# elador/FeatureDetection

Hardware: AMD Instinct MI355X
Metric: Mpatches/s (extract+WVM+SVM) per GPU, 640x480 pyramid (higher is better)
Workload: dtype u8/i32/f32/f64; 1 GPU; config 1/metric config: ffpDetectApp FaceFrontal.cfg five-stage cascade on 640x480 BGR frames: 13-layer pyramid, 20x20 windows step 1 (16185 windows/frame), HistEq64 -> WVM 280 filters -> OE -> RBF-SVM 1024 SV -> NMS; fd_pyramid_update_frames + fd_detect_five_stage_frames (the frames of a call share one pyramid aren...; frames_per_call=64, calls_in_flight=11, parallelism=image-shard dp1

## Files before the change

### featuredetection_amd/capi.py

```python
import ctypes as C
import os
import numpy as np

_HERE = os.path.dirname(os.path.abspath(__file__))
LIB_PATH = os.environ.get("FD_HIP_LIB", os.path.join(_HERE, "libfd_hip.so"))

FD_OK, FD_ERR_INVALID_ARGUMENT, FD_ERR_RUNTIME, FD_ERR_LOGIC, FD_ERR_HIP, FD_ERR_CAPACITY, FD_ERR_DEVICE_CAPACITY = range(7)
FD_LAYER_NONE, FD_LAYER_GRADBIN, FD_LAYER_LBP = 0, 1, 2
IMAGE_GRAY, IMAGE_GREYWORLD_GRAY = 0, 1
FD_KERNEL_LINEAR, FD_KERNEL_POLY, FD_KERNEL_RBF, FD_KERNEL_HIK = 0, 1, 2, 3
FD_DTYPE_U8, FD_DTYPE_F32 = 0, 1


class FdError(RuntimeError):
    def __init__(self, code, msg):
        super().__init__("fd_hip error %d: %s" % (code, msg))
        self.code = code


class fd_wvm_model(C.Structure):
    _fields_ = [("filter_w", C.c_int32), ("filter_h", C.c_int32), ("num_filters", C.c_int32), ("num_used", C.c_int32),
                ("num_per_level", C.c_int32), ("basis_param", C.c_float), ("bias", C.c_float),
                ("thresholds", C.POINTER(C.c_float)), ("hk_weights", C.POINTER(C.c_float)), ("pp", C.POINTER(C.c_double)),
                ("val_off", C.POINTER(C.c_int32)), ("val", C.POINTER(C.c_double)), ("rec_off", C.POINTER(C.c_int32)),
# ... 310 lines not shown
    "fd_integral_update": (C.c_int, [C.c_void_p, C.c_void_p, C.c_int, C.c_int, C.c_int, C.c_int]),
    "fd_integral_set_image": (C.c_int, [C.c_void_p, C.c_void_p, C.c_int, C.c_int]),
    "fd_integral_size": (C.c_int, [C.c_void_p, C.POINTER(C.c_int), C.POINTER(C.c_int)]),
    "fd_integral_download": (C.c_int, [C.c_void_p, C.c_void_p]),
    "fd_integral_image": (C.c_int, [C.c_void_p, C.c_void_p, C.c_int, C.c_int, C.c_void_p]),
    "fd_haar_grid": (C.c_int, [C.c_int, C.c_void_p]),
    "fd_haar_feature_count": (C.c_int, [C.POINTER(fd_haar_params)]),
    "fd_haar_features": (C.c_int, [C.POINTER(fd_haar_params), C.c_void_p, C.c_int, C.POINTER(C.c_int)]),
    "fd_integral_extract_haar": (C.c_int, [C.c_void_p, C.c_void_p, C.POINTER(fd_haar_params), C.c_int, C.c_void_p, C.c_void_p, C.c_void_p]),
    "fd_integral_gradient_patches": (C.c_int, [C.c_void_p, C.c_void_p, C.c_int, C.c_int, C.c_int, C.c_void_p, C.c_void_p, C.c_void_p]),
    "fd_gradient_sum_batch": (C.c_int, [C.c_void_p, C.c_void_p, C.c_int64, C.c_int, C.c_int, C.c_int, C.c_int, C.c_void_p]),
    "fd_integral_extract_surf": (C.c_int, [C.c_void_p, C.c_void_p, C.c_int, C.c_int, C.c_int, C.c_void_p, C.c_void_p, C.c_void_p]),
    "fd_integral_svm_evaluate_samples": (C.c_int, [C.c_void_p, C.c_void_p, C.c_int, C.c_void_p, C.c_void_p, C.c_int, C.c_void_p, C.c_void_p,
                                                   C.c_void_p]),
    "fd_integral_image_length": (C.c_int, [C.c_int, C.c_int]),
    "fd_integral_gradient_length": (C.c_int, [C.c_int, C.c_int]),
    "fd_gradient_sum_length": (C.c_int, [C.c_int, C.c_int, C.c_int, C.c_int]),
    "fd_surf_feature_length": (C.c_int, [C.c_int, C.c_int]),
}

_BENCH_SIGS = {
    "fd_debug_svm_u8_both": (C.c_int, [C.c_void_p, C.c_void_p, C.c_void_p, C.c_int64, C.c_void_p, C.c_void_p]),
    "fd_ctx_set_kernel_timing": (C.c_int, [C.c_void_p, C.c_int]),
    "fd_last_kernel_ms": (C.c_int, [C.c_void_p, C.POINTER(C.c_char_p), C.POINTER(C.c_float)]),
    "fd_last_group_prefilter_ms": (C.c_int, [C.c_void_p, C.POINTER(C.c_float), C.POINTER(C.c_int)]),
    "fd_debug_wvb_rect_sums": (C.c_int64, [C.POINTER(fd_wvm_model), C.c_void_p, C.c_int64, C.c_void_p, C.c_void_p]),
    "fd_wvm_last_queue_length": (C.c_int64, [C.c_void_p]),
    "fd_wvm_last_tail_state": (C.c_int, [C.c_void_p]),
    "fd_wvm_last_spec_state": (C.c_int, [C.c_void_p]),
    "fd_wvm_last_stage_b_plan": (C.c_int, [C.c_void_p, C.c_void_p]),
    "fd_debug_wvd_plan": (C.c_int, [C.c_void_p, C.c_void_p, C.c_int, C.c_int, C.c_int, C.c_int, C.c_int, C.c_void_p]),
    "fd_debug_wvd_packed_plan": (C.c_int, [C.c_void_p, C.c_void_p, C.c_int, C.c_int, C.c_int, C.c_int, C.c_int, C.c_void_p, C.c_void_p, C.c_void_p,
                                           C.c_int64, C.c_void_p]),
}


def lib():
    global _lib
    if _lib is None:
        if not os.path.exists(LIB_PATH):
            raise ImportError("%s not built: run `python -c 'import __graft_entry__ as g; g.build()'` "
                              "(hipcc --offload-arch=gfx950); there is no CPU fallback" % LIB_PATH)
        l = C.CDLL(LIB_PATH)
        for name, (res, args) in list(_SIGS.items()) + list(_BENCH_SIGS.items()):
            f = getattr(l, name)
            f.restype = res
            f.argtypes = args
        _lib = l
    return _lib


def _ptr(a):
    return a.ctypes.data_as(C.c_void_p) if a is not None else None


def _c(arr, dtype):
    return np.ascontiguousarray(arr, dtype=dtype)


class Context:
    def __init__(self, device=0, stream=None):
        self.h = C.c_void_p()
        rc = lib().fd_ctx_create(device, C.c_void_p(stream) if stream else None, C.byref(self.h))
        if rc != FD_OK:
            raise FdError(rc, "fd_ctx_create failed (no usable gfx950 device?)")

# ... 265 lines not shown
    dist.ctx.check(lib().fd_dist_gather_records(dist.h, _ptr(local), len(local), cap, None, 0, C.byref(n), C.byref(tr)))
    return int(n.value)


def svm_u8_both(ctx, svm, feats):
    feats = _c(feats, np.uint8).reshape(-1, svm.dim)
    o8, o16 = np.empty(len(feats), np.float64), np.empty(len(feats), np.float64)
    ctx.check(lib().fd_debug_svm_u8_both(ctx.h, svm.h, _ptr(feats), len(feats), _ptr(o8), _ptr(o16)))
    return o8, o16


def wvd_plan(nx, ny, frames, sy, ph, slots):
    nx, ny = _c(nx, np.int32), _c(ny, np.int32)
    first = np.zeros(len(nx) + 1, np.int32)
    k = lib().fd_debug_wvd_plan(_ptr(nx), _ptr(ny), len(nx), frames, sy, ph, slots, _ptr(first))
    if k < 1:
        raise FdError(k, "fd_debug_wvd_plan")
    return k, first


def wvd_packed_plan(nx, ny, frames, sy, ph, slots, tasks=None):
    nx, ny = _c(nx, np.int32), _c(ny, np.int32)
    tiles, ntask = C.c_int32(), C.c_int32()
    k = lib().fd_debug_wvd_packed_plan(_ptr(nx), _ptr(ny), len(nx), frames, sy, ph, slots, C.byref(tiles), C.byref(ntask), None, 0, None)
    if k < 1:
        raise FdError(k, "fd_debug_wvd_packed_plan")
    tasks = np.arange(ntask.value, dtype=np.int32) if tasks is None else _c(tasks, np.int32)
    dec = np.zeros((len(tasks), 4), np.int32)
    if len(tasks):
        k = lib().fd_debug_wvd_packed_plan(_ptr(nx), _ptr(ny), len(nx), frames, sy, ph, slots, None, None, _ptr(tasks), len(tasks), _ptr(dec))
        if k < 1:
            raise FdError(k, "fd_debug_wvd_packed_plan")
    return k, tiles.value, ntask.value, dec


def wvb_rect_sums(model, patches_eq):
    s, keep = _wvm_struct(model, fd_wvm_model)
    patches_eq = _c(patches_eq, np.uint8)
    n = patches_eq.shape[0]
    gen = np.zeros(5, np.int32)
    ncols = lib().fd_debug_wvb_rect_sums(C.byref(s), None, 0, None, _ptr(gen))
    if ncols < 0:
        return None
    out = np.empty((n, ncols), np.int32)
    lib().fd_debug_wvb_rect_sums(C.byref(s), _ptr(patches_eq), n, _ptr(out), None)
    return out, [int(g) for g in gen if g >= 0]


def wvm_eval(ctx, wvm, patches_eq):
    patches_eq = _c(patches_eq, np.uint8)
    n = patches_eq.shape[0]
    lv = np.empty(n, np.int32)
    sc = np.empty(n, np.float32)
    ctx.check(lib().fd_wvm_eval_batch(ctx.h, wvm.h, _ptr(patches_eq), n, _ptr(lv), _ptr(sc)))
    return lv, sc


class Svm:
    def __init__(self, ctx, model):
        self.ctx = ctx
        self.model = model
        dtype = np.uint8 if model["dtype"] == FD_DTYPE_U8 else np.float32
        sv = _c(model["sv"], dtype)
        coeff = _c(model["coeff"], np.float32)
        s = fd_svm_model()
        s.kernel = int(model["kernel"])
# ... 1193 lines not shown
```

### featuredetection_amd/csrc/pyramid.hip

```cpp
#include "fd_internal.hpp"
#include "fd_device.hpp"
#include <algorithm>
#include <cstring>

namespace {

constexpr int MAXJ = 16;

struct ResizeJob {
    int dw, dh;
    uint32_t dst_off;
    double scale_x, scale_y;
};
struct ResizeJobs {
    int n;
    ResizeJob j[MAXJ];
};
struct DownJob {
    int sw, sh;
    uint32_t src_off, dst_off;
};
struct FusedJob {
    int dw0, dh0, dw1, dh1;
    uint32_t dst0_off;
    uint32_t dst1_off;
    uint32_t xtab;
    double scale_y;
};
struct FusedJobs {
    int n;
    FusedJob j[MAXJ];
};
struct DownJobs {
    int n;
    int tile0[MAXJ + 1];
    DownJob j[MAXJ];
};
struct FilterJob {
    int w, h;
    uint32_t src_off, dst_off;
};
struct FilterJobs {
    int n;
    FilterJob j[MAXJ];
};

__device__ __forceinline__ int reflect101(int p, int len) {
    if (len == 1) return 0;
    while (p < 0 || p >= len) {
        if (p < 0) p = -p;
        else p = 2 * len - 2 - p;
    }
    return p;
}
__device__ __forceinline__ int reflect1(int p, int len) {
    if (len < 3) return reflect101(p, len);
    const int q = p < 0 ? -p : (p >= len ? 2 * len - 2 - p : p);
    return min(max(q, 0), len - 1);
}

struct FramePtrs {
    const uint8_t* p[FD_MAX_FRAMES];
};
__device__ __forceinline__ unsigned int mul24(unsigned int a, unsigned int b) {
    unsigned int r;
    asm("v_mul_u32_u24 %0, %1, %2" : "=v"(r) : "v"(a), "v"(b));
    return r;
}
__device__ __forceinline__ unsigned int mul24_s(unsigned int a_uniform, unsigned int b) {
    unsigned int r;
// ... 42 lines not shown
            uint32_t w[GQ][3];
#pragma unroll
            for (int i = 0; i < GQ; ++i) load3(min(q + i * stride, nq - 1), w[i]);
#pragma unroll
            for (int i = 0; i < GQ; ++i)
                if (q + i * stride < nq) reinterpret_cast<uint32_t*>(gray)[q + i * stride] = gray4(w[i]);
        } else {
            uint32_t w[GQ];
#pragma unroll
            for (int i = 0; i < GQ; ++i) w[i] = ld_u32_unaligned(src + 4 * (size_t)min(q + i * stride, nq - 1));
#pragma unroll
            for (int i = 0; i < GQ; ++i)
                if (q + i * stride < nq) reinterpret_cast<uint32_t*>(gray)[q + i * stride] = w[i];
        }
    }
    if (blockIdx.x == 0 && (int)threadIdx.x < (n & 3)) {
        const int i = (nq << 2) + threadIdx.x;
        gray[i] = ch == 3 ? (uint8_t)gray_of(src[3 * (size_t)i], src[3 * (size_t)i + 1], src[3 * (size_t)i + 2]) : src[i];
    }
}

__global__ void k_bgr2gray(const uint8_t* __restrict__ bgr, uint8_t* __restrict__ gray, int n) {
    int i = blockIdx.x * blockDim.x + threadIdx.x;
    int stride = gridDim.x * blockDim.x;
    for (; i < n; i += stride) {
        int b = bgr[3 * (size_t)i], g = bgr[3 * (size_t)i + 1], r = bgr[3 * (size_t)i + 2];
        gray[i] = (uint8_t)((b * 1868 + g * 9617 + r * 4899 + 8192) >> 14);
    }
}

constexpr int TL_W = 64, TL_H = 32, TL_PITCH = 136;
constexpr int PD_TH = 16;
constexpr int TL_ROWS = 72;

__global__ __launch_bounds__(256) void k_resize_tiled(const uint8_t* __restrict__ arena, uint8_t* __restrict__ out, uint32_t src_off, int sw,
                                                      int sh, ResizeJobs jobs, size_t imageStride) {
    __shared__ __attribute__((aligned(16))) uint8_t tile[TL_ROWS * TL_PITCH];
    __shared__ int4 rowTab[TL_H];
    const ResizeJob jb = jobs.j[blockIdx.y];
    const uint8_t* src = arena + (size_t)blockIdx.z * imageStride + src_off;
    uint8_t* dst = out + (size_t)blockIdx.z * imageStride + jb.dst_off;
    const int tilesX = (jb.dw + TL_W - 1) / TL_W, tilesY = (jb.dh + TL_H - 1) / TL_H;
    auto srcX = [&](int dx, float& fx) {
        fx = (float)((dx + 0.5) * jb.scale_x - 0.5);
        int sx = (int)floorf(fx);
        fx -= sx;
        if (sx < 0) { fx = 0; sx = 0; }
        if (sx >= sw - 1) { fx = 0; sx = sw - 1; }
        return sx;
    };
    auto srcY = [&](int dy, float& fy) {
        fy = (float)((dy + 0.5) * jb.scale_y - 0.5);
        const int sy = (int)floorf(fy);
        fy -= sy;
        return sy;
    };
    auto clampY = [&](int y) { return y < 0 ? 0 : (y >= sh ? sh - 1 : y); };
    const int c = threadIdx.x & 63, rq = __builtin_amdgcn_readfirstlane(threadIdx.x >> 6);
    for (int t = blockIdx.x; t < tilesX * tilesY; t += gridDim.x) {
        const int ty = t / tilesX, tx = t - ty * tilesX;
        const int dx0 = tx * TL_W, dy0 = ty * TL_H;
        const int X0 = max(0, (int)((float)dx0 * (float)jb.scale_x) - 1), Y0 = max(0, (int)((float)dy0 * (float)jb.scale_y) - 1);
        {
            const int x = X0 + 4 * c;
            const bool colok = c < TL_PITCH / 4;
            uint32_t v[TL_ROWS / 4];
// ... 130 lines not shown
        if (itemN < items)
            fused_issue(f, arena0 + (size_t)frame_of(itemN) * imageStride + src_off, sw, sh, tabs, jobs.j[dN.w], dN);
        PYR_T(p3);
        {
            const int c = threadIdx.x & 127, half = __builtin_amdgcn_readfirstlane(threadIdx.x >> 7);
            if (c < G0_W) {
                const int rBase = half * (G0_H - 18);
                const int lx = min(max(ex.x - X0, 0), FS_PITCH - 1) + 2 * rBase * FS_PITCH;
                int lx1 = lx + 1;
                asm("" : "+v"(lx1));
                const uint8_t *sp = stage + lx, *sp1 = stage + lx1;
                const uint2* tp = taps + rBase;
                const u16x2 aw = __builtin_bit_cast(u16x2, ex.y);
                uint8_t* gp = g0 + rBase * G0_PITCH + c;
#pragma unroll
                for (int i = 0; i < 18; ++i) {
                    const uint8_t *s = sp + 2 * i * FS_PITCH, *s1 = sp1 + 2 * i * FS_PITCH;
                    const u16x2 p0 = {s[0], s1[0]}, p1 = {s[FS_PITCH], s1[FS_PITCH]};
                    const uint2 t = tp[i];
                    const unsigned int h0 = __builtin_amdgcn_udot2(p0, aw, 0u, false) & ~15u;
                    const unsigned int h1 = __builtin_amdgcn_udot2(p1, aw, 0u, false) & ~15u;
                    gp[i * G0_PITCH] = (uint8_t)((mulhi24(t.x, h0) + mulhi24(t.y, h1) + 2) >> 2);
                }
            }
        }
        PYR_T(p4);
        __syncthreads();
        PYR_T(p5);
        {
            const int c1 = lane;
            const int x = x1 + c1;
            if (c1 < FT_W1 && x < jb.dw1) {
                constexpr int PR = FT_H1 / 4;
                const uint8_t* T = g0 + (2 * wave * PR) * G0_PITCH + 2 * c1;
                int h[2 * PR + 3];
#pragma unroll
                for (int r = 0; r < 2 * PR + 3; ++r) {
                    const uint8_t* S = T + r * G0_PITCH;
                    const uint32_t p01 = *reinterpret_cast<const uint16_t*>(S), p23 = *reinterpret_cast<const uint16_t*>(S + 2);
                    h[r] = (int)__builtin_amdgcn_udot4(p01 | (p23 << 16), 0x04060401u, (uint32_t)S[4], false);
                }
                uint8_t* dp = arena + jb.dst1_off + (uint32_t)((y1 + wave * PR) * jb.dw1) + x;
#pragma unroll
                for (int j = 0; j < PR; ++j, dp += jb.dw1) {
                    if (y1 + wave * PR + j < jb.dh1) {
                        const int v = h[2 * j + 2] * 6 + (h[2 * j + 1] + h[2 * j + 3]) * 4 + h[2 * j] + h[2 * j + 4];
                        *dp = (uint8_t)((v + 128) >> 8);
                    }
                }
            }
        }
        if (jb.dst0_off != 0xffffffffu) {
            uint8_t* d0 = arena + jb.dst0_off;
            for (int i = threadIdx.x; i < 32 * 128; i += 256) {
                const int r = 2 + (i >> 7), c = 2 + (i & 127);
                const int gx = gx0 + c, gy = gy0 + r;
                if (c < 2 + 2 * FT_W1 && gx < jb.dw0 && gy < jb.dh0) d0[(uint32_t)(gy * jb.dw0) + gx] = g0[r * G0_PITCH + c];
            }
        }
#ifdef FD_PYR_PROF
        {
            const unsigned long long p6 = __builtin_amdgcn_s_memtime();
            pacc[0] += p1 - p0; pacc[1] += p2 - p1; pacc[2] += p3 - p2; pacc[3] += p4 - p3; pacc[4] += p5 - p4; pacc[5] += p6 - p5; ++ptiles;
        }
#endif
    }
#ifdef FD_PYR_PROF
    if (threadIdx.x == 0 && blockIdx.x < (unsigned int)PYR_PROF_WGS) {
        for (int i = 0; i < 6; ++i) fd_pyr_prof[blockIdx.x * 8 + i] = pacc[i];
        fd_pyr_prof[blockIdx.x * 8 + 6] = ptiles;
    }
#endif
}

__device__ __forceinline__ int reflect_cf(int p, int len) {
    int q = p < 0 ? -p : p;
    q = q >= len ? 2 * len - 2 - q : q;
    return min(max(q, 0), len - 1);
}
constexpr int PD_W = 62;
__global__ __launch_bounds__(256) void k_pyrdown_tiled(uint8_t* __restrict__ arena0, DownJobs jobs, size_t imageStride, int xcdFrames) {
    __shared__ __attribute__((aligned(16))) uint8_t tile[TL_ROWS * TL_PITCH];
    const int c = threadIdx.x & 63, rq = __builtin_amdgcn_readfirstlane(threadIdx.x >> 6);
    constexpr int NROWS = 2 * PD_TH + 3, PD_LD = (NROWS + 7) / 8;
    static_assert(2 * (3 + 4 * (PD_LD - 1)) + 1 < TL_ROWS && 128 <= TL_PITCH && 2 * PD_W + 3 <= 128, "pyrDown stage");
    const bool byXcd = xcdFrames > 0;
    const int ntile = jobs.tile0[jobs.n];
    const int first = byXcd ? (int)(blockIdx.x >> 3) : (int)blockIdx.x, stride = byXcd ? (int)(gridDim.x >> 3) : (int)gridDim.x;
    const int items = byXcd ? (xcdFrames >> 3) * ntile : ntile;
    for (int item = first; item < items; item += stride) {
        const int fi = byXcd ? item / ntile : 0;
        const int g = item - fi * ntile;
        uint8_t* __restrict__ arena = arena0 + (size_t)(byXcd ? (int)(blockIdx.x & 7u) + 8 * fi : (int)blockIdx.z) * imageStride;
        int ji = 0;
        while (ji + 1 < jobs.n && g >= jobs.tile0[ji + 1]) ++ji;
        const DownJob jb = jobs.j[ji];
        const int t = g - jobs.tile0[ji];
        const int sw = jb.sw, sh = jb.sh;
        const int dw = (sw + 1) / 2, dh = (sh + 1) / 2;
        const uint8_t* src = arena + jb.src_off;
        uint8_t* dst = arena + jb.dst_off;
        const int tilesX = (dw + PD_W - 1) / PD_W;
        const int ty = t / tilesX, tx = t - ty * tilesX;
        const int dx0 = tx * PD_W, dy0 = ty * PD_TH;
        const int X0 = 2 * dx0 - 2, Y0 = 2 * dy0 - 2;
        {
            const int j4 = 4 * (c & 31), half = c >> 5;
            const int xs = X0 + j4;
            const int xc = min(max(xs, 0), max(sw - 4, 0));
            const uint32_t lastDw = (uint32_t)max(sw * sh - 4, 0);
            uint32_t v[PD_LD];
#pragma unroll
            for (int k = 0; k < PD_LD; ++k) {
                const int r = 2 * (rq + 4 * k) + half;
                v[k] = ld_u32_unaligned(src + min((uint32_t)(reflect_cf(Y0 + r, sh) * sw + xc), lastDw));
            }
            if (X0 < 0 || X0 + 128 > sw) {
                if (!(xs >= 0 && xs + 3 < sw)) {
#pragma unroll
                    for (int k = 0; k < PD_LD; ++k) {
                        const int r = 2 * (rq + 4 * k) + half;
                        const uint8_t* row = src + (uint32_t)(reflect_cf(Y0 + r, sh) * sw);
                        uint32_t w = 0;
#pragma unroll
                        for (int b = 0; b < 4; ++b) w |= (uint32_t)row[reflect_cf(xs + b, sw)] << (8 * b);
                        v[k] = w;
                    }
                }
            }
#pragma unroll
            for (int k = 0; k < PD_LD; ++k) *reinterpret_cast<uint32_t*>(&tile[(2 * (rq + 4 * k) + half) * TL_PITCH + j4]) = v[k];
        }
        __syncthreads();
        const int x = dx0 + c;
        if (c < PD_W && x < dw) {
            constexpr int PR = PD_TH / 4;
            const uint8_t* T = tile + (2 * rq * PR) * TL_PITCH + 2 * c;
            int h[2 * PR + 3];
#pragma unroll
            for (int r = 0; r < 2 * PR + 3; ++r) {
                const uint8_t* S = T + r * TL_PITCH;
                const uint32_t p01 = *reinterpret_cast<const uint16_t*>(S), p23 = *reinterpret_cast<const uint16_t*>(S + 2);
                h[r] = (int)__builtin_amdgcn_udot4(p01 | (p23 << 16), 0x04060401u, (uint32_t)S[4], false);
            }
            uint8_t* dp = dst + (uint32_t)((dy0 + rq * PR) * dw) + x;
#pragma unroll
            for (int j = 0; j < PR; ++j, dp += dw) {
                if (dy0 + rq * PR + j < dh) {
                    const int v = h[2 * j + 2] * 6 + (h[2 * j + 1] + h[2 * j + 3]) * 4 + h[2 * j] + h[2 * j + 4];
                    *dp = (uint8_t)((v + 128) >> 8);
                }
            }
        }
        __syncthreads();
    }
}

__device__ __forceinline__ float grad_pair(const uint8_t* __restrict__ src, int w, int h, int x, int y, int ksize, int& gx, int& gy) {
    if (ksize == 1 || ksize == 3) {
        const int xm = reflect101(x - 1, w), xp = reflect101(x + 1, w);
        const int ym = reflect101(y - 1, h), yp = reflect101(y + 1, h);
        const uint8_t *S0 = src + (size_t)ym * w, *S1 = src + (size_t)y * w, *S2 = src + (size_t)yp * w;
        if (ksize == 1) {
            gx = S1[xp] - S1[xm];
            gy = S2[x] - S0[x];
            return 0.5f;
        }
        gx = (S0[xp] - S0[xm]) + 2 * (S1[xp] - S1[xm]) + (S2[xp] - S2[xm]);
        gy = (S2[xm] - S0[xm]) + 2 * (S2[x] - S0[x]) + (S2[xp] - S0[xp]);
        return 0.125f;
    }
    int a, d1, d2, d3, s0, s1, s2, s3;
    float scale;
    if (ksize == 5) { a = 2; d1 = 2; d2 = 1; d3 = 0; s0 = 6; s1 = 4; s2 = 1; s3 = 0; scale = 1.f / 128.f; }
    else if (ksize == 7) { a = 3; d1 = 5; d2 = 4; d3 = 1; s0 = 20; s1 = 15; s2 = 6; s3 = 1; scale = 1.f / 2048.f; }
    else { a = 1; d1 = 1; d2 = 0; d3 = 0; s0 = 10; s1 = 3; s2 = 0; s3 = 0; scale = 1.f / 32.f; }
    const int dk[4] = {0, d1, d2, d3}, sk[4] = {s0, s1, s2, s3};
    int cx[7], cy[7];
    for (int t = -a; t <= a; ++t) { cx[t + a] = reflect101(x + t, w); cy[t + a] = reflect101(y + t, h); }
    gx = 0;
    gy = 0;
    for (int j = -a; j <= a; ++j) {
        const uint8_t* S = src + (size_t)cy[j + a] * w;
        int rd = 0, rs = 0;
        for (int i = 1; i <= a; ++i) {
            const int hi = S[cx[a + i]], lo = S[cx[a - i]];
            rd += dk[i] * (hi - lo);
// ... 292 lines not shown
                if (direction < 0) direction += PI;
                bin = direction * bins / PI;
            }
            auto sat = [](double v) { int r = fd_cvRound(v); return (uint8_t)(r < 0 ? 0 : (r > 255 ? 255 : r)); };
            size_t index = (size_t)x | ((size_t)y << 8);
            if (!interpolate) {
                lut[2 * index] = (uint8_t)((uint8_t)std::round(bin) % (unsigned)bins);
                lut[2 * index + 1] = sat(255 * magnitude);
            } else {
                uint8_t w1 = sat(255 * magnitude * (bin - std::floor(bin)));
                lut[4 * index] = (uint8_t)((uint8_t)std::floor(bin) % (unsigned)bins);
                lut[4 * index + 1] = sat(255 * magnitude - w1);
                lut[4 * index + 2] = (uint8_t)((uint8_t)std::ceil(bin) % (unsigned)bins);
                lut[4 * index + 3] = w1;
            }
        }
    }
}

int grid_for(int npix) { return std::max(1, std::min(1024, (npix + 255) / 256)); }
int tile_grid_for(int ntiles) { return std::max(1, std::min(1024, ntiles)); }

struct ResizeLaunch {
    ResizeJobs jobs;
    int grid;
};
struct FusedLaunch {
    FusedJobs jobs;
    uint32_t tileTab;
    int tilesPerFrame;
    int grid;
};
struct DownLaunch {
    DownJobs jobs;
};
struct FilterLaunch {
    FilterJobs jobs, blur;
    int grid;
};

}

struct fd_pyramid::Plan {
    std::vector<ResizeLaunch> resize;
    std::vector<FusedLaunch> fused;
    std::vector<DownLaunch> down;
    std::vector<FilterLaunch> filter;
};
fd_pyramid::~fd_pyramid() { if (ready) (void)hipEventDestroy(ready); }

namespace {

template <class Launch>
auto& next_job(std::vector<Launch>& launches, size_t first = 0) {
    if (launches.size() == first || launches.back().jobs.n == MAXJ) launches.emplace_back();
    auto& jobs = launches.back().jobs;
    return jobs.j[jobs.n++];
}

void build_plan(fd_pyramid* p, int W, int H) {
    p->plan.reset(new fd_pyramid::Plan());
    fd_pyramid::Plan& plan = *p->plan;
    const std::vector<HostLayer>& all = p->all;
    const int NI = p->nimg;
    static const int mode = [] { const char* e = getenv("FD_PYR_FUSED"); return e ? atoi(e) : 1; }();
    std::vector<char> fused(all.size(), 0);
    std::vector<int2> tab;
    std::vector<std::vector<int4>> tiles;
    for (size_t k = 0; k < all.size(); ++k) {
        const HostLayer& L = all[k];
        if (L.depth != 0) continue;
        if (L.w == W && L.h == H && L.gray_off == p->gray_full_off) continue;
        const double scale_x = 1. / ((double)L.w / W), scale_y = 1. / ((double)L.h / H);
        if (!(scale_x >= 1.0 && scale_x <= 2.05 && scale_y >= 1.0 && scale_y <= 2.05))
            FD_THROW(FD_ERR_RUNTIME, "ImagePyramid: first-octave layer %d x %d of a %d x %d image is outside the resize kernel's range", L.w, L.h, W, H);
        const bool chain = k + 1 < all.size() && all[k + 1].depth == 1 && all[k + 1].chain == L.chain;
        if (chain && mode != 0 && (!L.kept || mode == 2) && L.w >= 3 && L.h >= 3 && W <= 65535 && H <= 65535) {
            const HostLayer& D = all[k + 1];
            std::vector<int2> xt((size_t)L.w);
            for (int dx = 0; dx < L.w; ++dx) {
                float fx = (float)((dx + 0.5) * scale_x - 0.5);
                int sx = (int)floorf(fx);
                fx -= sx;
                if (sx < 0) { fx = 0; sx = 0; }
                if (sx >= W - 1) { fx = 0; sx = W - 1; }
                const int a0 = (int)nearbyintf((1.f - fx) * 2048), a1 = (int)nearbyintf(fx * 2048);
                xt[(size_t)dx] = make_int2(sx, a0 | (a1 << 16));
            }
// ... 11 lines not shown
                j.scale_y = scale_y;
                tab.insert(tab.end(), xt.begin(), xt.end());
                tiles.resize(plan.fused.size());
                for (int ty = 0; ty * FT_H1 < D.h; ++ty)
                    for (int tx = 0; tx * FT_W1 < D.w; ++tx) {
                        const int gx0 = 2 * tx * FT_W1 - 2;
                        const int cLo = std::max(0, gx0), cHi = std::min(L.w - 1, gx0 + G0_W - 1);
                        const int X0 = xt[(size_t)cLo].x, ncol = std::min(W - 1, xt[(size_t)cHi].x + 1) - X0 + 1;
                        tiles.back().push_back(make_int4(X0, ncol, (int)((uint32_t)tx | (uint32_t)ty << 16), plan.fused.back().jobs.n - 1));
                    }
                fused[k] = 1;
                continue;
            }
        }
        ResizeJob& j = next_job(plan.resize);
        j.dw = L.w; j.dh = L.h; j.dst_off = L.gray_off;
        j.scale_x = scale_x;
        j.scale_y = scale_y;
        ResizeLaunch& R = plan.resize.back();
        R.grid = std::max(R.grid, tile_grid_for(((L.w + TL_W - 1) / TL_W) * ((L.h + TL_H - 1) / TL_H)));
    }
    if (!plan.fused.empty()) {
        int perCu = 0;
        if (hipOccupancyMaxActiveBlocksPerMultiprocessor(&perCu, k_resize_down, 256, 0) != hipSuccess || perCu < 1) perCu = 4;
        for (size_t g = 0; g < plan.fused.size(); ++g) {
            FusedLaunch& F = plan.fused[g];
            if (tab.size() & 1) tab.push_back(make_int2(0, 0));
            F.tileTab = (uint32_t)tab.size();
            F.tilesPerFrame = (int)tiles[g].size();
            for (const int4& t : tiles[g]) { tab.push_back(make_int2(t.x, t.y)); tab.push_back(make_int2(t.z, t.w)); }
            F.grid = (int)std::min<int64_t>((int64_t)F.tilesPerFrame * NI, (int64_t)p->ctx->num_cus * perCu);
            if (NI >= 8 && F.grid >= 64) F.grid &= ~7;
        }
        p->rtab.reserve(sizeof(int2) * tab.size());
        HIP_CHECK(hipMemcpy(p->rtab.p, tab.data(), sizeof(int2) * tab.size(), hipMemcpyHostToDevice));
    }
    int maxDepth = 0;
    for (const HostLayer& L : all) maxDepth = std::max(maxDepth, L.depth);
    for (int d = 1; d <= maxDepth; ++d) {
        const size_t first = plan.down.size();
        for (size_t k = 1; k < all.size(); ++k) {
            const HostLayer& L = all[k];
            if (L.depth != d || fused[k - 1]) continue;
            const HostLayer& S = all[k - 1];
            DownJob& j = next_job(plan.down, first);
            j.sw = S.w; j.sh = S.h; j.src_off = S.gray_off; j.dst_off = L.gray_off;
            DownJobs& jobs = plan.down.back().jobs;
            jobs.tile0[jobs.n] = jobs.tile0[jobs.n - 1] + ((L.w + PD_W - 1) / PD_W) * ((L.h + PD_TH - 1) / PD_TH);
        }
    }
    if (p->filter_kind != FD_LAYER_NONE) {
        const bool blur = p->filter_kind == FD_LAYER_GRADBIN && p->grad_blur > 0;
        for (int k : p->kept) {
            const HostLayer& L = all[k];
            FilterJob& j = next_job(plan.filter);
            j.w = L.w; j.h = L.h; j.src_off = blur ? L.blur_off : L.gray_off; j.dst_off = L.filt_off;
            FilterLaunch& F = plan.filter.back();
            if (blur) {
                FilterJob& b = F.blur.j[F.blur.n++];
                b.w = L.w; b.h = L.h; b.src_off = L.gray_off; b.dst_off = L.blur_off;
            }
            F.grid = std::max(F.grid, grid_for(L.w * L.h));
        }
    }
}

void invalidate_layout(fd_pyramid* p) {
    p->all.clear();
    p->img_w = p->img_h = 0;
}

void build_layout(fd_pyramid* p, int W, int H) {
    invalidate_layout(p);
    p->kept.clear();
    size_t off = 0;
    p->gray_full_off = 0;
    off = align256((size_t)W * H);
    const int fch = p->filter_kind == FD_LAYER_GRADBIN ? (p->interpolate ? 4 : 2) : 1;
    for (size_t i = 0; i < p->octl; ++i) {
        double scaleFactor = std::pow(p->inc, (double)i);
        int w = fd_cvRound(W * scaleFactor), h = fd_cvRound(H * scaleFactor);
        if (w < 1 || h < 1) FD_THROW(FD_ERR_INVALID_ARGUMENT, "ImagePyramid: layer %zu would be empty", i);
// ... 65 lines not shown
    const size_t IS = p->image_stride;
    FramePtrs fp{};
    if (!is_device) p->input.reserve(bytes * NI);
    for (int f = 0; f < NI; ++f) {
        fp.p[f] = frames ? frames[f] : image;
        if (!is_device) {
            uint8_t* staged = p->input.as<uint8_t>() + (size_t)f * bytes;
            HIP_CHECK(hipMemcpyAsync(staged, fp.p[f], bytes, hipMemcpyHostToDevice, st));
            fp.p[f] = staged;
        }
    }
    if (greyworld) {
        GwStats* stats = p->gw_stats.as<GwStats>();
        HIP_CHECK(hipMemsetAsync(stats, 0, sizeof(GwStats) * (size_t)NI, st));
        const int cus = std::max(1, p->ctx->num_cus);
        const int perFrame = std::max(1, std::min(cus, 4 * cus / NI));
        const int gx = std::max(1, std::min((int)((npix / 4 + 1023) / 1024), perFrame));
        hipLaunchKernelGGL(k_gw_stats, dim3(gx, NI), dim3(256), 0, st, fp, stats, (int)npix);
        hipLaunchKernelGGL(k_gw_gray, dim3(gx, NI), dim3(256), 0, st, fp, stats, gray, IS, (int)npix);
    } else if (frames) {
        hipLaunchKernelGGL(k_frames_to_gray, dim3(grid_for((int)(npix / 16 + 1)), NI), dim3(256), 0, st, fp, gray, IS, (int)npix, ch);
    } else if (ch == 3) {
        hipLaunchKernelGGL(k_bgr2gray, dim3(grid_for((int)npix)), dim3(256), 0, st, fp.p[0], gray, (int)npix);
    } else {
        HIP_CHECK(hipMemcpyAsync(gray, fp.p[0], npix, hipMemcpyDeviceToDevice, st));
    }
    const fd_pyramid::Plan& plan = *p->plan;
    for (const ResizeLaunch& R : plan.resize)
        hipLaunchKernelGGL(k_resize_tiled, dim3(R.grid, R.jobs.n, NI), dim3(256), 0, st, arena, arena, p->gray_full_off, W, H, R.jobs, IS);
    for (const FusedLaunch& F : plan.fused)
        hipLaunchKernelGGL(k_resize_down, dim3(F.grid), dim3(256), 0, st, arena, p->gray_full_off, W, H, p->rtab.as<int2>(), F.jobs, F.tileTab, F.tilesPerFrame, NI, IS);
    const bool downByXcd = NI >= 8 && NI % 8 == 0 && fd_knob_pyr_xcd();
    for (const DownLaunch& D : plan.down) {
        const int ntile = D.jobs.tile0[D.jobs.n];
        if (downByXcd)
            hipLaunchKernelGGL(k_pyrdown_tiled, dim3(8 * (int)std::min<int64_t>((int64_t)(NI / 8) * ntile, 8192)), dim3(256), 0, st, arena, D.jobs, IS, NI);
        else
            hipLaunchKernelGGL(k_pyrdown_tiled, dim3(tile_grid_for(ntile), 1, NI), dim3(256), 0, st, arena, D.jobs, IS, 0);
    }
    for (const FilterLaunch& F : plan.filter) {
        const dim3 g(F.grid, F.jobs.n);
        if (F.blur.n) hipLaunchKernelGGL(k_box_blur, g, dim3(256), 0, st, arena, p->grad_blur, F.blur);
        if (p->filter_kind != FD_LAYER_GRADBIN)
            hipLaunchKernelGGL(k_lbp, g, dim3(256), 0, st, arena, p->lbp_type, F.jobs);
        else if (p->interpolate)
            hipLaunchKernelGGL(k_gradbin<4>, g, dim3(256), 0, st, arena, p->lut.as<uint8_t>(), p->grad_kernel, F.jobs);
        else
            hipLaunchKernelGGL(k_gradbin<2>, g, dim3(256), 0, st, arena, p->lut.as<uint8_t>(), p->grad_kernel, F.jobs);
    }
    HIP_CHECK(hipGetLastError());
    if (!p->ready) HIP_CHECK(hipEventCreateWithFlags(&p->ready, hipEventDisableTiming));
    HIP_CHECK(hipEventRecord(p->ready, st));
    p->readyStream = st;
    p->version++;
}

}

void fd_pyramid_update_on(fd_pyramid* p, const uint8_t* image, int w, int h, int ch, int is_device, hipStream_t st) {
    if (!p) FD_THROW(FD_ERR_INVALID_ARGUMENT, "fd_pyramid_update: NULL pyramid");
    HIP_CHECK(hipSetDevice(p->ctx->device));
    pyramid_update(p, image, w, h, ch, is_device, st);
}

void fd_enumerate_layers(const fd_pyramid* p, int pw, int ph, int sx, int sy, const int* roiIn,
                         std::vector<WindowLayer>& out, int64_t& total) {
    if (sx < 1) FD_THROW(FD_ERR_INVALID_ARGUMENT, "DirectPyramidFeatureExtractor: stepX has to be greater than zero");
    if (sy < 1) FD_THROW(FD_ERR_INVALID_ARGUMENT, "DirectPyramidFeatureExtractor: stepY has to be greater than zero");
    if (pw < 1 || ph < 1) FD_THROW(FD_ERR_INVALID_ARGUMENT, "DirectPyramidFeatureExtractor: empty patch size");
    int rx = 0, ry = 0, rw = 0, rh = 0;
    if (!roiIn && p->sel_has_roi) roiIn = p->sel_roi;
// ... 324 lines not shown
        DevBuf in, out, dl;
        in.reserve(2 * n);
        out.reserve((size_t)E * n);
        dl.reserve(lut.size());
        HIP_CHECK(hipMemcpyAsync(dl.p, lut.data(), lut.size(), hipMemcpyHostToDevice, ctx->stream));
        HIP_CHECK(hipMemcpyAsync(in.p, grad2ch, 2 * n, hipMemcpyHostToDevice, ctx->stream));
        if (E == 2) hipLaunchKernelGGL(k_binning_image<2>, dim3(grid_for((int)n)), dim3(256), 0, ctx->stream, in.as<uint8_t>(), dl.as<uint8_t>(), out.as<uint8_t>(), (int)n);
        else hipLaunchKernelGGL(k_binning_image<4>, dim3(grid_for((int)n)), dim3(256), 0, ctx->stream, in.as<uint8_t>(), dl.as<uint8_t>(), out.as<uint8_t>(), (int)n);
        HIP_CHECK(hipGetLastError());
        HIP_CHECK(hipMemcpyAsync(dst, out.p, (size_t)E * n, hipMemcpyDeviceToHost, ctx->stream));
        HIP_CHECK(hipStreamSynchronize(ctx->stream));
    });
}

int fd_lbp_image(fd_ctx* ctx, const uint8_t* gray, int w, int h, int lbp_type, uint8_t* dst) {
    return fd_guard(ctx, [&] {
        if (!ctx || !gray || !dst || w < 1 || h < 1) FD_THROW(FD_ERR_INVALID_ARGUMENT, "fd_lbp_image: bad argument");
        if (lbp_type < 0 || lbp_type > 3) FD_THROW(FD_ERR_INVALID_ARGUMENT, "LbpFilter: invalid type");
        HIP_CHECK(hipSetDevice(ctx->device));
        const size_t n = (size_t)w * h, doff = (n + 255) & ~(size_t)255;
        DevBuf buf;
        buf.reserve(doff + n);
        HIP_CHECK(hipMemcpyAsync(buf.p, gray, n, hipMemcpyHostToDevice, ctx->stream));
        FilterJobs jobs;
        jobs.n = 1;
        jobs.j[0].w = w; jobs.j[0].h = h; jobs.j[0].src_off = 0; jobs.j[0].dst_off = (uint32_t)doff;
        hipLaunchKernelGGL(k_lbp, dim3(grid_for((int)n), 1), dim3(256), 0, ctx->stream, buf.as<uint8_t>(), lbp_type, jobs);
        HIP_CHECK(hipGetLastError());
        HIP_CHECK(hipMemcpyAsync(dst, buf.as<uint8_t>() + doff, n, hipMemcpyDeviceToHost, ctx->stream));
        HIP_CHECK(hipStreamSynchronize(ctx->stream));
    });
}

}

#ifdef FD_PYR_PROF
extern "C" int fd_debug_pyr_prof(unsigned long long* out) {
    if (out) (void)hipMemcpyFromSymbol(out, HIP_SYMBOL(fd_pyr_prof), sizeof(unsigned long long) * 8 * PYR_PROF_WGS);
    return PYR_PROF_WGS;
}
#endif
```

### include/fd_hip_bench.h

```cpp
#ifndef FD_HIP_BENCH_H_
#define FD_HIP_BENCH_H_
#include "fd_hip.h"
#ifdef __cplusplus
extern "C" {
#endif

int fd_ctx_set_kernel_timing(fd_ctx* ctx, int enable);
int fd_last_kernel_ms(fd_ctx* ctx, const char** kernel_name, float* ms);
int fd_last_group_prefilter_ms(fd_ctx* ctx, float* ms, int* members);

int64_t fd_wvm_last_queue_length(const fd_wvm* wvm);
int fd_wvm_last_stage_b_plan(const fd_wvm* wvm, int64_t* out);
int fd_wvm_last_tail_state(const fd_wvm* wvm);
int fd_wvm_last_spec_state(const fd_wvm* wvm);

int64_t fd_debug_wvb_rect_sums(const fd_wvm_model* md, const uint8_t* patches, int64_t n, int32_t* out, int32_t* phase_gen);

int fd_debug_wvd_plan(const int32_t* nx, const int32_t* ny, int n_layers, int frames, int sy, int ph, int slots, int32_t* tile_first);

int fd_debug_wvd_packed_plan(const int32_t* nx, const int32_t* ny, int n_layers, int frames, int sy, int ph, int slots, int32_t* tiles_per_frame,
                             int32_t* tasks_per_frame, const int32_t* tasks, int64_t n_tasks, int32_t* decoded);

int fd_debug_svm_u8_both(fd_ctx* ctx, const fd_svm* svm, const uint8_t* features, int64_t n, double* out8, double* out16);

#ifdef __cplusplus
}
#endif
#endif
```

Baseline: 3893 Mpatches/s.

## Precompute pyrDown tile table on host and simplify tiled pyrDown kernel

Replaces the per-launch DownJobs struct with a device-side table of precomputed per-tile entries (offsets, origin, extent). Each block now handles exactly one tile instead of grid-striding and scanning the job prefix. Staging uses a clamped 4-byte load plus a byte permute for edge columns instead of a branchy fallback, and uses a smaller LDS tile. The shared column-filter helper is factored out and reused by the fused resize kernel. The goal is less scalar address math and divergence in the pyramid build, at the cost of an extra global table read per block and a larger grid.

New measurement: 4099 Mpatches/s (median of 6 runs). 5.3% higher.

```diff
diff --git a/featuredetection_amd/capi.py b/featuredetection_amd/capi.py
--- a/featuredetection_amd/capi.py
+++ b/featuredetection_amd/capi.py
@@ -366,6 +366,7 @@
     "fd_debug_wvd_plan": (C.c_int, [C.c_void_p, C.c_void_p, C.c_int, C.c_int, C.c_int, C.c_int, C.c_int, C.c_void_p]),
     "fd_debug_wvd_packed_plan": (C.c_int, [C.c_void_p, C.c_void_p, C.c_int, C.c_int, C.c_int, C.c_int, C.c_int, C.c_void_p, C.c_void_p, C.c_void_p,
                                            C.c_int64, C.c_void_p]),
+    "fd_debug_pyrdown_stage": (C.c_int, [C.c_void_p, C.c_int, C.c_int, C.c_int, C.c_void_p, C.c_void_p]),
 }
 
 
@@ -697,6 +698,21 @@
         if k < 1:
             raise FdError(k, "fd_debug_wvd_packed_plan")
     return k, tiles.value, ntask.value, dec
+
+
+def pyrdown_stage(image, tile):
+    image = _c(image, np.uint8)
+    sh, sw = image.shape
+    if tile is None:
+        nt = lib().fd_debug_pyrdown_stage(None, sw, sh, 0, None, None)
+        if nt < 1:
+            raise FdError(1, "fd_debug_pyrdown_stage: no such tile")
+        return nt
+    staged, entry = np.zeros((35, 128), np.uint8), np.zeros(8, np.int32)
+    nt = lib().fd_debug_pyrdown_stage(_ptr(image), sw, sh, tile, _ptr(staged), _ptr(entry))
+    if nt < 1:
+        raise FdError(1, "fd_debug_pyrdown_stage: no such tile")
+    return nt, staged, dict(zip(("src_off", "dst_off", "sw", "sh", "dx0", "dy0", "nx", "ny"), entry.tolist()))
 
 
 def wvb_rect_sums(model, patches_eq):
diff --git a/featuredetection_amd/csrc/pyramid.hip b/featuredetection_amd/csrc/pyramid.hip
--- a/featuredetection_amd/csrc/pyramid.hip
+++ b/featuredetection_amd/csrc/pyramid.hip
@@ -15,10 +15,6 @@
 struct ResizeJobs {
     int n;
     ResizeJob j[MAXJ];
-};
-struct DownJob {
-    int sw, sh;
-    uint32_t src_off, dst_off;
 };
 struct FusedJob {
     int dw0, dh0, dw1, dh1;
@@ -31,11 +27,14 @@
     int n;
     FusedJob j[MAXJ];
 };
-struct DownJobs {
-    int n;
-    int tile0[MAXJ + 1];
-    DownJob j[MAXJ];
+struct PdTile {
+    uint32_t src_off;
+    uint32_t dst_off;
+    int sw, sh;
+    int dx0, dy0;
+    int nx, ny;
 };
+static_assert(sizeof(PdTile) == 32, "a tile entry is eight dwords");
 struct FilterJob {
     int w, h;
     uint32_t src_off, dst_off;
@@ -144,6 +143,22 @@
 constexpr int TL_W = 64, TL_H = 32, TL_PITCH = 136;
 constexpr int PD_TH = 16;
 constexpr int TL_ROWS = 72;
+
+typedef const __attribute__((address_space(3))) uint8_t* lds_bytes;
+template <int PITCH>
+__device__ __forceinline__ void pyrdown_col4(lds_bytes T, uint32_t out[4]) {
+    uint32_t h[11];
+#pragma unroll
+    for (int r = 0; r < 11; ++r) {
+        lds_bytes S = T + r * PITCH;
+        typedef const __attribute__((address_space(3))) uint16_t* lds_u16;
+        const uint32_t p01 = *(lds_u16)S, p23 = *(lds_u16)(S + 2);
+        h[r] = __builtin_amdgcn_udot4(p01 | (p23 << 16), 0x04060401u, (uint32_t)S[4], false);
+    }
+#pragma unroll
+    for (int j = 0; j < 4; ++j)
+        out[j] = (mad24(h[2 * j + 2], 6u, ((h[2 * j + 1] + h[2 * j + 3]) << 2) + h[2 * j]) + h[2 * j + 4] + 128u) >> 8;
+}
 
 __global__ __launch_bounds__(256) void k_resize_tiled(const uint8_t* __restrict__ arena, uint8_t* __restrict__ out, uint32_t src_off, int sw,
                                                       int sh, ResizeJobs jobs, size_t imageStride) {
@@ -340,22 +355,13 @@
             const int x = x1 + c1;
             if (c1 < FT_W1 && x < jb.dw1) {
                 constexpr int PR = FT_H1 / 4;
-                const uint8_t* T = g0 + (2 * wave * PR) * G0_PITCH + 2 * c1;
-                int h[2 * PR + 3];
-#pragma unroll
-                for (int r = 0; r < 2 * PR + 3; ++r) {
-                    const uint8_t* S = T + r * G0_PITCH;
-                    const uint32_t p01 = *reinterpret_cast<const uint16_t*>(S), p23 = *reinterpret_cast<const uint16_t*>(S + 2);
-                    h[r] = (int)__builtin_amdgcn_udot4(p01 | (p23 << 16), 0x04060401u, (uint32_t)S[4], false);
-                }
+                static_assert(PR == 4, "pyrdown_col4");
+                uint32_t v[PR];
+                pyrdown_col4<G0_PITCH>((lds_bytes)g0 + (2 * wave * PR) * G0_PITCH + 2 * c1, v);
                 uint8_t* dp = arena + jb.dst1_off + (uint32_t)((y1 + wave * PR) * jb.dw1) + x;
 #pragma unroll
-                for (int j = 0; j < PR; ++j, dp += jb.dw1) {
-                    if (y1 + wave * PR + j < jb.dh1) {
-                        const int v = h[2 * j + 2] * 6 + (h[2 * j + 1] + h[2 * j + 3]) * 4 + h[2 * j] + h[2 * j + 4];
-                        *dp = (uint8_t)((v + 128) >> 8);
-                    }
-                }
+                for (int j = 0; j < PR; ++j, dp += jb.dw1)
+                    if (y1 + wave * PR + j < jb.dh1) *dp = (uint8_t)v[j];
             }
         }
         if (jb.dst0_off != 0xffffffffu) {
@@ -381,86 +387,104 @@
 #endif
 }
 
-__device__ __forceinline__ int reflect_cf(int p, int len) {
+constexpr int PD_W = 62;
+constexpr int PD_LD = 5;
+constexpr int PD_ROWS = 8 * PD_LD;
+constexpr int PD_PITCH = 136;
+static_assert(2 * PD_TH + 3 <= PD_ROWS && 2 * PD_W + 3 <= 128 && 128 <= PD_PITCH, "pyrDown stage");
+
+__host__ __device__ inline int reflect_cf(int p, int len) {
     int q = p < 0 ? -p : p;
     q = q >= len ? 2 * len - 2 - q : q;
-    return min(max(q, 0), len - 1);
-}
-constexpr int PD_W = 62;
-__global__ __launch_bounds__(256) void k_pyrdown_tiled(uint8_t* __restrict__ arena0, DownJobs jobs, size_t imageStride, int xcdFrames) {
-    __shared__ __attribute__((aligned(16))) uint8_t tile[TL_ROWS * TL_PITCH];
+    q = q < 0 ? 0 : q;
+    return q > len - 1 ? len - 1 : q;
+}
+__host__ __device__ inline int pd_tiles(int sw, int sh) { return (((sw + 1) / 2 + PD_W - 1) / PD_W) * (((sh + 1) / 2 + PD_TH - 1) / PD_TH); }
+__host__ __device__ inline PdTile pd_tile_entry(int sw, int sh, uint32_t src_off, uint32_t dst_off, int t) {
+    const int dw = (sw + 1) / 2, dh = (sh + 1) / 2, tilesX = (dw + PD_W - 1) / PD_W;
+    const int ty = t / tilesX, tx = t - ty * tilesX;
+    PdTile e;
+    e.src_off = src_off;
+    e.sw = sw; e.sh = sh;
+    e.dx0 = tx * PD_W; e.dy0 = ty * PD_TH;
+    e.dst_off = dst_off + (uint32_t)(e.dy0 * dw + e.dx0);
+    e.nx = dw - e.dx0 < PD_W ? dw - e.dx0 : PD_W;
+    e.ny = dh - e.dy0 < PD_TH ? dh - e.dy0 : PD_TH;
+    return e;
+}
+struct PdCol {
+    int xc;
+    uint32_t sel;
+};
+__host__ __device__ inline PdCol pd_col(int xs, int sw) {
+    PdCol pc;
+    pc.xc = xs < 0 ? 0 : (xs > sw - 4 ? sw - 4 : xs);
+    const int d = xs - pc.xc;
+    const uint32_t right = (uint32_t)(0x0000010203020100ull >> (8 * ((d > 5 ? 5 : d) & 7)));
+    pc.sel = d < 0 ? 0x01000102u : right;
+    return pc;
+}
+__host__ __device__ inline uint32_t pd_perm(uint32_t v, uint32_t sel) {
+#ifdef __HIP_DEVICE_COMPILE__
+    return __builtin_amdgcn_perm(v, v, sel);
+#else
+    uint32_t r = 0;
+    for (int i = 0; i < 4; ++i) r |= ((v >> (8 * ((sel >> (8 * i)) & 3u))) & 0xffu) << (8 * i);
+    return r;
+#endif
+}
+__host__ __device__ inline void pd_stage(const uint8_t* __restrict__ src, const PdTile& e, int rq, int lane, uint32_t v[PD_LD]) {
+    const int sw = e.sw, sh = e.sh;
+    const int xs = 2 * e.dx0 - 2 + 4 * (lane & 31), Y0 = 2 * e.dy0 - 2 + 2 * rq;
+    const uint32_t odd = 0u - (uint32_t)(lane >> 5);
+    if (sw >= 8) {
+        const PdCol pc = pd_col(xs, sw);
+#pragma unroll
+        for (int k = 0; k < PD_LD; ++k) {
+            const uint32_t o0 = (uint32_t)(reflect_cf(Y0 + 8 * k, sh) * sw), o1 = (uint32_t)(reflect_cf(Y0 + 8 * k + 1, sh) * sw);
+            uint32_t w;
+            __builtin_memcpy(&w, src + (o0 + ((o1 - o0) & odd) + (uint32_t)pc.xc), 4);
+            v[k] = pd_perm(w, pc.sel);
+        }
+    } else {
+#pragma unroll
+        for (int k = 0; k < PD_LD; ++k) {
+            const uint8_t* row = src + (uint32_t)(reflect_cf(Y0 + 8 * k + (int)(odd & 1u), sh) * sw);
+            uint32_t w = 0;
+            for (int b = 0; b < 4; ++b) w |= (uint32_t)row[reflect_cf(xs + b, sw)] << (8 * b);
+            v[k] = w;
+        }
+    }
+}
+
+__global__ __launch_bounds__(256) void k_pyrdown_tiled(uint8_t* __restrict__ arena0, const PdTile* __restrict__ tiles, size_t imageStride, int xcdShift) {
+    __shared__ __attribute__((aligned(16))) uint8_t tile[PD_ROWS * PD_PITCH];
     const int c = threadIdx.x & 63, rq = __builtin_amdgcn_readfirstlane(threadIdx.x >> 6);
-    constexpr int NROWS = 2 * PD_TH + 3, PD_LD = (NROWS + 7) / 8;
-    static_assert(2 * (3 + 4 * (PD_LD - 1)) + 1 < TL_ROWS && 128 <= TL_PITCH && 2 * PD_W + 3 <= 128, "pyrDown stage");
-    const bool byXcd = xcdFrames > 0;
-    const int ntile = jobs.tile0[jobs.n];
-    const int first = byXcd ? (int)(blockIdx.x >> 3) : (int)blockIdx.x, stride = byXcd ? (int)(gridDim.x >> 3) : (int)gridDim.x;
-    const int items = byXcd ? (xcdFrames >> 3) * ntile : ntile;
-    for (int item = first; item < items; item += stride) {
-        const int fi = byXcd ? item / ntile : 0;
-        const int g = item - fi * ntile;
-        uint8_t* __restrict__ arena = arena0 + (size_t)(byXcd ? (int)(blockIdx.x & 7u) + 8 * fi : (int)blockIdx.z) * imageStride;
-        int ji = 0;
-        while (ji + 1 < jobs.n && g >= jobs.tile0[ji + 1]) ++ji;
-        const DownJob jb = jobs.j[ji];
-        const int t = g - jobs.tile0[ji];
-        const int sw = jb.sw, sh = jb.sh;
-        const int dw = (sw + 1) / 2, dh = (sh + 1) / 2;
-        const uint8_t* src = arena + jb.src_off;
-        uint8_t* dst = arena + jb.dst_off;
-        const int tilesX = (dw + PD_W - 1) / PD_W;
-        const int ty = t / tilesX, tx = t - ty * tilesX;
-        const int dx0 = tx * PD_W, dy0 = ty * PD_TH;
-        const int X0 = 2 * dx0 - 2, Y0 = 2 * dy0 - 2;
-        {
-            const int j4 = 4 * (c & 31), half = c >> 5;
-            const int xs = X0 + j4;
-            const int xc = min(max(xs, 0), max(sw - 4, 0));
-            const uint32_t lastDw = (uint32_t)max(sw * sh - 4, 0);
-            uint32_t v[PD_LD];
-#pragma unroll
-            for (int k = 0; k < PD_LD; ++k) {
-                const int r = 2 * (rq + 4 * k) + half;
-                v[k] = ld_u32_unaligned(src + min((uint32_t)(reflect_cf(Y0 + r, sh) * sw + xc), lastDw));
-            }
-            if (X0 < 0 || X0 + 128 > sw) {
-                if (!(xs >= 0 && xs + 3 < sw)) {
-#pragma unroll
-                    for (int k = 0; k < PD_LD; ++k) {
-                        const int r = 2 * (rq + 4 * k) + half;
-                        const uint8_t* row = src + (uint32_t)(reflect_cf(Y0 + r, sh) * sw);
-                        uint32_t w = 0;
-#pragma unroll
-                        for (int b = 0; b < 4; ++b) w |= (uint32_t)row[reflect_cf(xs + b, sw)] << (8 * b);
-                        v[k] = w;
-                    }
-                }
-            }
-#pragma unroll
-            for (int k = 0; k < PD_LD; ++k) *reinterpret_cast<uint32_t*>(&tile[(2 * (rq + 4 * k) + half) * TL_PITCH + j4]) = v[k];
-        }
-        __syncthreads();
-        const int x = dx0 + c;
-        if (c < PD_W && x < dw) {
-            constexpr int PR = PD_TH / 4;
-            const uint8_t* T = tile + (2 * rq * PR) * TL_PITCH + 2 * c;
-            int h[2 * PR + 3];
-#pragma unroll
-            for (int r = 0; r < 2 * PR + 3; ++r) {
-                const uint8_t* S = T + r * TL_PITCH;
-                const uint32_t p01 = *reinterpret_cast<const uint16_t*>(S), p23 = *reinterpret_cast<const uint16_t*>(S + 2);
-                h[r] = (int)__builtin_amdgcn_udot4(p01 | (p23 << 16), 0x04060401u, (uint32_t)S[4], false);
-            }
-            uint8_t* dp = dst + (uint32_t)((dy0 + rq * PR) * dw) + x;
-#pragma unroll
-            for (int j = 0; j < PR; ++j, dp += dw) {
-                if (dy0 + rq * PR + j < dh) {
-                    const int v = h[2 * j + 2] * 6 + (h[2 * j + 1] + h[2 * j + 3]) * 4 + h[2 * j] + h[2 * j + 4];
-                    *dp = (uint8_t)((v + 128) >> 8);
-                }
-            }
-        }
-        __syncthreads();
+    const uint32_t frame = (blockIdx.x & ((1u << xcdShift) - 1u)) + 8u * blockIdx.y + blockIdx.z;
+    const PdTile e = tiles[blockIdx.x >> xcdShift];
+    uint8_t* __restrict__ arena = arena0 + (size_t)frame * imageStride;
+    {
+        uint32_t v[PD_LD];
+        pd_stage(arena + e.src_off, e, rq, c, v);
+        uint8_t* sp = tile + 2 * rq * PD_PITCH + ((0u - (uint32_t)(c >> 5)) & (uint32_t)PD_PITCH) + 4 * (c & 31);
+#pragma unroll
+        for (int k = 0; k < PD_LD; ++k) *reinterpret_cast<uint32_t*>(sp + 8 * k * PD_PITCH) = v[k];
+    }
+    __syncthreads();
+    if (c < e.nx) {
+        constexpr int PR = PD_TH / 4;
+        static_assert(PR == 4, "pyrdown_col4");
+        uint32_t v[PR];
+        pyrdown_col4<PD_PITCH>((lds_bytes)tile + (2 * rq * PR) * PD_PITCH + 2 * c, v);
+        const int dw = (e.sw + 1) >> 1;
+        uint8_t* dst = arena + e.dst_off + (uint32_t)(rq * PR * dw);
+#pragma unroll
+        for (int j = 0; j < PR; ++j, dst += dw)
+            if (rq * PR + j < e.ny) {
+                uint32_t col = (uint32_t)c;
+                asm("" : "+v"(col));
+                dst[col] = (uint8_t)v[j];
+            }
     }
 }
 
@@ -819,7 +843,9 @@
     int grid;
 };
 struct DownLaunch {
-    DownJobs jobs;
+    int njobs;
+    int ntile;
+    uint32_t tileTab;
 };
 struct FilterLaunch {
     FilterJobs jobs, blur;
@@ -839,8 +865,8 @@
 namespace {
 
 template <class Launch>
-auto& next_job(std::vector<Launch>& launches, size_t first = 0) {
-    if (launches.size() == first || launches.back().jobs.n == MAXJ) launches.emplace_back();
+auto& next_job(std::vector<Launch>& launches) {
+    if (launches.empty() || launches.back().jobs.n == MAXJ) launches.emplace_back();
     auto& jobs = launches.back().jobs;
     return jobs.j[jobs.n++];
 }
@@ -918,22 +944,35 @@
             F.grid = (int)std::min<int64_t>((int64_t)F.tilesPerFrame * NI, (int64_t)p->ctx->num_cus * perCu);
             if (NI >= 8 && F.grid >= 64) F.grid &= ~7;
         }
-        p->rtab.reserve(sizeof(int2) * tab.size());
-        HIP_CHECK(hipMemcpy(p->rtab.p, tab.data(), sizeof(int2) * tab.size(), hipMemcpyHostToDevice));
     }
     int maxDepth = 0;
     for (const HostLayer& L : all) maxDepth = std::max(maxDepth, L.depth);
+    static_assert(sizeof(PdTile) == 4 * sizeof(int2), "PdTile entries in rtab");
     for (int d = 1; d <= maxDepth; ++d) {
         const size_t first = plan.down.size();
         for (size_t k = 1; k < all.size(); ++k) {
             const HostLayer& L = all[k];
             if (L.depth != d || fused[k - 1]) continue;
             const HostLayer& S = all[k - 1];
-            DownJob& j = next_job(plan.down, first);
-            j.sw = S.w; j.sh = S.h; j.src_off = S.gray_off; j.dst_off = L.gray_off;
-            DownJobs& jobs = plan.down.back().jobs;
-            jobs.tile0[jobs.n] = jobs.tile0[jobs.n - 1] + ((L.w + PD_W - 1) / PD_W) * ((L.h + PD_TH - 1) / PD_TH);
-        }
+            if (plan.down.size() == first || plan.down.back().njobs == MAXJ) {
+                if (tab.size() & 1) tab.push_back(make_int2(0, 0));
+                plan.down.push_back(DownLaunch{0, 0, (uint32_t)tab.size()});
+            }
+            DownLaunch& D = plan.down.back();
+            const int nt = pd_tiles(S.w, S.h);
+            for (int t = 0; t < nt; ++t) {
+                const PdTile e = pd_tile_entry(S.w, S.h, S.gray_off, L.gray_off, t);
+                int2 q[4];
+                std::memcpy(q, &e, sizeof(e));
+                tab.insert(tab.end(), q, q + 4);
+            }
+            D.njobs++;
+            D.ntile += nt;
+        }
+    }
+    if (!tab.empty()) {
+        p->rtab.reserve(sizeof(int2) * tab.size());
+        HIP_CHECK(hipMemcpy(p->rtab.p, tab.data(), sizeof(int2) * tab.size(), hipMemcpyHostToDevice));
     }
     if (p->filter_kind != FD_LAYER_NONE) {
         const bool blur = p->filter_kind == FD_LAYER_GRADBIN && p->grad_blur > 0;
@@ -1065,11 +1104,11 @@
         hipLaunchKernelGGL(k_resize_down, dim3(F.grid), dim3(256), 0, st, arena, p->gray_full_off, W, H, p->rtab.as<int2>(), F.jobs, F.tileTab, F.tilesPerFrame, NI, IS);
     const bool downByXcd = NI >= 8 && NI % 8 == 0 && fd_knob_pyr_xcd();
     for (const DownLaunch& D : plan.down) {
-        const int ntile = D.jobs.tile0[D.jobs.n];
+        const PdTile* tiles = reinterpret_cast<const PdTile*>(p->rtab.as<int2>() + D.tileTab);
         if (downByXcd)
-            hipLaunchKernelGGL(k_pyrdown_tiled, dim3(8 * (int)std::min<int64_t>((int64_t)(NI / 8) * ntile, 8192)), dim3(256), 0, st, arena, D.jobs, IS, NI);
+            hipLaunchKernelGGL(k_pyrdown_tiled, dim3(8 * D.ntile, NI / 8), dim3(256), 0, st, arena, tiles, IS, 3);
         else
-            hipLaunchKernelGGL(k_pyrdown_tiled, dim3(tile_grid_for(ntile), 1, NI), dim3(256), 0, st, arena, D.jobs, IS, 0);
+            hipLaunchKernelGGL(k_pyrdown_tiled, dim3(D.ntile, 1, NI), dim3(256), 0, st, arena, tiles, IS, 0);
     }
     for (const FilterLaunch& F : plan.filter) {
         const dim3 g(F.grid, F.jobs.n);
@@ -1460,6 +1499,27 @@
     });
 }
 
+int fd_debug_pyrdown_stage(const uint8_t* image, int sw, int sh, int tile, uint8_t* staged, int32_t* entry) {
+    if (sw < 1 || sh < 1 || (int64_t)sw * sh > 0x7fffffff) return -1;
+    const int nt = pd_tiles(sw, sh);
+    if (!image && !staged && !entry) return nt;
+    if (!image || tile < 0 || tile >= nt) return -1;
+    const PdTile e = pd_tile_entry(sw, sh, 0, 0, tile);
+    if (entry) std::memcpy(entry, &e, sizeof(e));
+    if (staged) {
+        for (int rq = 0; rq < 4; ++rq)
+            for (int lane = 0; lane < 64; ++lane) {
+                uint32_t v[PD_LD];
+                pd_stage(image, e, rq, lane, v);
+                for (int k = 0; k < PD_LD; ++k) {
+                    const int r = 2 * (rq + 4 * k) + (lane >> 5);
+                    if (r < 2 * PD_TH + 3) std::memcpy(staged + r * 128 + 4 * (lane & 31), &v[k], 4);
+                }
+            }
+    }
+    return nt;
+}
+
 }
 
 #ifdef FD_PYR_PROF
diff --git a/include/fd_hip_bench.h b/include/fd_hip_bench.h
--- a/include/fd_hip_bench.h
+++ b/include/fd_hip_bench.h
@@ -21,6 +21,8 @@
 int fd_debug_wvd_packed_plan(const int32_t* nx, const int32_t* ny, int n_layers, int frames, int sy, int ph, int slots, int32_t* tiles_per_frame,
                              int32_t* tasks_per_frame, const int32_t* tasks, int64_t n_tasks, int32_t* decoded);
 
+int fd_debug_pyrdown_stage(const uint8_t* image, int sw, int sh, int tile, uint8_t* staged, int32_t* entry);
+
 int fd_debug_svm_u8_both(fd_ctx* ctx, const fd_svm* svm, const uint8_t* features, int64_t n, double* out8, double* out16);
 
 #ifdef __cplusplus
```
